# DHDev0/Stochastic-muzero

Hardware: AMD Instinct MI355X
Metric: MCTS simulations/sec (whole node), CartPole MLP 4096 envs × 50 sims (higher is better)
Workload: dtype f32 (tree values, heads) + f64 (pUCT scores, root priors) + i32 (counts)

## Files before the change

stochastic-muzero_amd/csrc/smz_kernels.hip:

```cpp
#ifndef SMZ_SEARCH_THREADS
#define SMZ_SEARCH_THREADS 512
#endif
#ifndef SMZ_EB_WAVES
#define SMZ_EB_WAVES 4
#endif
#ifndef SMZ_PAIR_K4
#define SMZ_PAIR_K4 1
#endif
#ifndef SMZ_KS4
#define SMZ_KS4 1
#endif
#ifndef SMZ_PART
#define SMZ_PART 0
#endif
#ifndef SMZ_PRIO_TREE
#define SMZ_PRIO_TREE 0
#define SMZ_PRIO_HEADS 3
#endif
#include <hip/hip_runtime.h>
#include <math.h>
#include <stdint.h>
#include <stdio.h>
#include <stdlib.h>
#include <string.h>
// ... 582 lines not shown
        r[0] = (double)(float)nx; r[1] = (double)(float)nxd; r[2] = (double)(float)nth; r[3] = (double)(float)nthd;
        r[4] = 1.0;
        r[5] = (double)flag;
        r[6] = policy[(size_t)e * A]; r[7] = policy[(size_t)e * A + 1];
        r[8] = act == 0 ? 1.0 : 0.0; r[9] = act == 1 ? 1.0 : 0.0;
        r[10] = (double)root_value[e];
        r[11] = child_visits[(size_t)e * A]; r[12] = child_visits[(size_t)e * A + 1];
    }
    if (E.reward_out) E.reward_out[e] = 1.0f;
    if (E.flag_out) E.flag_out[e] = (uint8_t)flag;
    int next_count = count;
    if (flag != 0 && E.on_end == 2) {
        const int ep = E.episode[e] + 1;
        E.episode[e] = ep;
        nx = -0.05 + 0.1 * smz_unit(E.reset_seed, (uint64_t)(E.first_env + e), (uint64_t)ep, 0);
        nxd = -0.05 + 0.1 * smz_unit(E.reset_seed, (uint64_t)(E.first_env + e), (uint64_t)ep, 1);
        nth = -0.05 + 0.1 * smz_unit(E.reset_seed, (uint64_t)(E.first_env + e), (uint64_t)ep, 2);
        nthd = -0.05 + 0.1 * smz_unit(E.reset_seed, (uint64_t)(E.first_env + e), (uint64_t)ep, 3);
        next_count = 0;
    } else if (flag != 0 && E.on_end == 1 && E.active) {
        E.active[e] = 0;
    }
    if (E.step_count) E.step_count[e] = next_count;
    st[0] = nx; st[1] = nxd; st[2] = nth; st[3] = nthd;
    if (E.obs_out) {
        float *o = E.obs_out + (size_t)e * 4;
        o[0] = (float)nx; o[1] = (float)nxd; o[2] = (float)nth; o[3] = (float)nthd;
    }
}

extern __shared__ float4 smz_search_lds4[];

#ifndef SMZ_BPS_HBM
#define SMZ_BPS_HBM 1
#endif
#ifndef SMZ_SELECT_BLOCKS
#define SMZ_SELECT_BLOCKS 1
#endif
#ifndef SMZ_EARLY_ROWS
#define SMZ_EARLY_ROWS 1
#endif
#ifndef SMZ_PAIR_A4
#define SMZ_PAIR_A4 1
#endif
#ifndef SMZ_SELECT_TWO_PASSES
#define SMZ_SELECT_TWO_PASSES 1
#endif
#ifndef SMZ_LEAF_FIRST
#define SMZ_LEAF_FIRST 1
#endif
#ifndef SMZ_EARLY_STAGE
#define SMZ_EARLY_STAGE 1
#endif
#ifdef SMZ_BPS_PROBE
#define SMZ_PROBE_DECL unsigned long long pb_t0 = 0, pb_acc[7] = {0, 0, 0, 0, 0, 0, 0};
#define SMZ_PROBE_START pb_t0 = __builtin_amdgcn_s_memtime();
#define SMZ_PROBE_AT(i) { const unsigned long long pb_t1 = __builtin_amdgcn_s_memtime(); pb_acc[i] += pb_t1 - pb_t0; pb_t0 = pb_t1; }
#if SMZ_BPS_PROBE + 0 == 2
#define SMZ_PROBE(i)
#define SMZ_PROBE_B(i) SMZ_PROBE_AT(i)
#else
#define SMZ_PROBE(i) SMZ_PROBE_AT(i)
#define SMZ_PROBE_B(i)
#endif
#define SMZ_PROBE_FLUSH(stats) if ((stats) && lane == 0) { for (int pb_i = 0; pb_i < 7; pb_i++) atomicAdd(&(stats)[8 + pb_i], pb_acc[pb_i]); }
#else
#define SMZ_PROBE_DECL
#define SMZ_PROBE_START
#define SMZ_PROBE(i)
#define SMZ_PROBE_B(i)
#define SMZ_PROBE_FLUSH(stats)
#endif

struct MegaLds {
    int pbc_off, wave_off, per_wave;
    int x_off, pv_off, rng_off, out_off, sel_off, sel_n;
    int sel_on;
    int trees_off, tree_words;
};
__host__ __device__ inline int r4(int x) { return (x + 3) & ~3; }
__host__ __device__ inline MegaLds mega_lds(const smz_mlp_desc &d, const Params &P, int tpw, bool tlds = false, int waves = 8) {
    MegaLds m;
    m.pbc_off = r4(tlds ? smz_mlp::compact_total_floats(d) : d.total_floats - smz_mlp::rep_floats(d));
    m.wave_off = m.pbc_off + r4(2 * 2 * (P.sims + 2));
    m.x_off = r4(2 * smz_mlp::row_scratch_floats(d));
    m.pv_off = m.x_off + tpw * smz_mlp::up4(P.S + P.A);
    m.rng_off = m.pv_off + tpw * P.P * 4;
    m.out_off = m.rng_off + r4(tpw * kRngStride);
    m.sel_off = m.out_off + r4(tpw * (P.A + 2));
    m.sel_n = (P.sims + 2 + 1) & ~1;
    bool sel = tlds;
    if (!tlds && SMZ_BPS_HBM && P.A == 2 && P.K == 2 && tpw == 2 && P.sims <= 126) {
        const int per = m.sel_off + r4(tpw * m.sel_n);
        sel = ((size_t)m.wave_off + (size_t)waves * per) * sizeof(float) <= (size_t)160 * 1024;
    }
    m.sel_on = sel ? 1 : 0;
    m.per_wave = m.sel_off + (sel ? r4(tpw * m.sel_n) : 0);
    m.tree_words = r4(P.rb_words + P.sims * 6 * P.K + (P.K == 2 ? 2 * P.sims : 0));
    m.trees_off = m.wave_off + waves * m.per_wave;
    return m;
}

struct ActOut {
    double temperature;
    int32_t *action;
    double *policy, *child_visits;
    float *root_value;
};
constexpr int kFastTpw = 2, kFastS = 31, kFastH = 64, kFastL = 0;
#if SMZ_PART == 0 || SMZ_PART == 2 || SMZ_PART == 4 || SMZ_PART == 6
template <int MAXA, int KS, int U, bool INSTR, bool AEX, bool MSK = true, bool PHX = false, bool TLDS = false>
__global__ void __launch_bounds__(SMZ_SEARCH_THREADS) k_search_mlp(Params Pin, smz_mlp_desc d, const float *weights, const float *obs,
                                                    int train, ActOut act, EnvStep env) {
    Params P = Pin;
    P.tree0 = 0;
    if (AEX) { P.A = MAXA; P.tpw = kFastTpw; d.A = MAXA; d.S = kFastS; d.H = kFastH; d.L = kFastL; d.OP = smz_mlp::kWave; P.S = kFastS; }
    if (AEX) P.philox = PHX ? 1 : 0;
    if (KS > 0) P.K = KS;
    fix_layout(P, AEX, KS > 0);
    if (AEX) P.hs = (kFastS + 15) & ~15;
    float *lds = reinterpret_cast<float *>(smz_search_lds4);
    static_assert(!TLDS || (AEX && KS > 0), "LDS-resident trees: the specialised instantiations only");
    const smz_mlp_desc dl = TLDS ? smz_mlp::lds_desc_compact(d) : smz_mlp::lds_desc_without_rep(d);
    if (TLDS) smz_mlp::stage_weights_compact(lds, weights, d);
    else smz_mlp::stage_weights_without_rep(lds, weights, d);
    const int lane = threadIdx.x & (kWave - 1), wave = threadIdx.x / kWave, waves = blockDim.x / kWave;
    const int A = P.A, S = P.S, tpw = P.tpw;
    const MegaLds ml = mega_lds(d, P, tpw, TLDS, waves);
    uint32_t *const nodes_global = P.nodes;
    const int gl_eb_words = P.eb_words;
    if (TLDS) {
        uint32_t *nodes_lds = reinterpret_cast<uint32_t *>(lds + ml.trees_off);
        for (int i = threadIdx.x; i < waves * tpw * ml.tree_words; i += blockDim.x) nodes_lds[i] = 0u;
        P.nodes = nodes_lds;
        P.tree0 = blockIdx.x * waves * tpw;
        P.eb_words = 6 * KS;
        P.tree_words = ml.tree_words;
    }
    constexpr bool THR = AEX && KS == 2, YV = THR && TLDS;
    if (THR) {
        P.thr_off = TLDS ? P.rb_words + P.sims * 6 * KS : P.rb_words + 12;
        P.thr_stride = TLDS ? 2 : P.eb_words;
        P.ry_off = (YV && MAXA <= 8 && P.rp_off + 3 * A <= P.rb_words) ? P.rp_off + 2 * A : -1;
    }
    double *pbc_lds = reinterpret_cast<double *>(lds + ml.pbc_off);
    const int n_pbc = P.sims + 2;
    for (int i = threadIdx.x; i < n_pbc; i += blockDim.x) {
        pbc_lds[i] = P.pbc_sqrt[i];
        pbc_lds[n_pbc + i] = i > 0 ? 1.0 / (double)i : 0.0;
    }
    const int slot = A + 2;
    const int K4in = smz_mlp::up4(S + A);
    float *scratch = lds + ml.wave_off + wave * ml.per_wave;
    float *xall = scratch + ml.x_off;
    uint4 *pvals = reinterpret_cast<uint4 *>(scratch + ml.pv_off);
    uint32_t *rng_tile = reinterpret_cast<uint32_t *>(scratch + ml.rng_off);
    float *outs = scratch + ml.out_off;
    __syncthreads();

    const int tree0 = (blockIdx.x * waves + wave) * tpw;
    const int tree = tree0 + lane;
    const bool valid = lane < tpw && tree < P.B && (!MSK || tree_active(P, tree));
    if (MSK && __ballot(valid) == 0ull) {
        if (env.state && lane < tpw && tree < P.B) cartpole_env_step(env, tree, P.B, act.action, act.policy, act.child_visits, act.root_value);
        return;
    }

    for (int t = 0; t < tpw; t++) {
        const int row = tree0 + t;
        if (row >= P.B) break;
        if (MSK && !__shfl((int)valid, t)) continue;
        smz_mlp::initial_row<U, TLDS>(lds, dl, weights, d, scratch, obs + (size_t)row * d.obs, P.hidden + (size_t)row * P.N * P.hs,
                                      nullptr, outs + t * slot);
    }
    constexpr bool PHC = !AEX || PHX;
    int packed = wave_stage_rng<PHC>(P, tree, valid, rng_tile);
    RngT<PHC> rng;
    rng.bind(P, tree, valid);
    TreeHdr h = {0, 0, 0.f, 0.f, 0, 0.f, 0, 0};
    if (valid) {
        rng.load(P.mt + (size_t)tree * kMtN, packed, rng_tile + lane * kRngStride, kRngStage);
        root_init_tree<MAXA>(P, tree, rng, outs + lane * slot, nullptr, train != 0);
        h = P.hdr[tree];
        packed = rng.pack();
    }
    unsigned n_dec = 0, n_chance = 0, n_children = 0, n_desc = 0;
    const int vmask = MSK ? __builtin_amdgcn_readlane((int)valid, 0) | (__builtin_amdgcn_readlane((int)valid, 1) << 1) : 3;
#define SMZ_SLOT_VALID(src) (MSK ? ((vmask >> (src)) & 1) != 0 : tree0 + (src) < P.B)
    const bool prof = INSTR && (P.dbg & 16) && P.stats;
    const int dbg = INSTR ? P.dbg : 0;
    unsigned long long t_stage = 0, t_expand = 0, t_select = 0, t_mlp = 0, t0 = 0, t1 = 0;
#define SMZ_STAMP(acc) if (INSTR && prof) { t1 = __builtin_amdgcn_s_memtime(); acc += t1 - t0; t0 = t1; }
    constexpr int SU = 2;
    const bool split = P.tpw <= SU;
    if (P.sims > 0 && !(dbg & 8)) packed = wave_stage_rng_from<4, PHC>(P, tree, valid, rng_tile, packed, rng.block());
    SMZ_PROBE_DECL
    for (int s = 0; s < P.sims; s++) {
        if (INSTR && prof) t0 = __builtin_amdgcn_s_memtime();
        SMZ_PROBE_START
        Leaf L = {0, 0, 0, 0};
        __builtin_amdgcn_s_setprio(SMZ_PRIO_TREE);
        constexpr bool LBKP = AEX && !INSTR;
        float leaf_rw = 0.f;
        if (valid) {
            rng.load(P.mt + (size_t)tree * kMtN, packed, rng_tile + lane * kRngStride, kRngStage);
            if (s > 0 && !(dbg & 4)) expand_backup_tree<MAXA, KS, LBKP, THR, YV>(P, tree, rng, h, outs + lane * slot, outs[lane * slot + A + 1],
                                                      outs[lane * slot + A], pvals + lane * P.P, &leaf_rw);
        }
        SMZ_PROBE_B(0)
        if constexpr (LBKP) {
            if (s > 0) {
                const int src = lane & (kFastTpw - 1);
                const int len = pick_lane01(h.path_len, src);
                const float lrw = pick_lane01(leaf_rw, src);
                if (lane < 8 * kFastTpw && SMZ_SLOT_VALID(src)) {
                    const bool own = lane < kFastTpw;
                    float mn = own ? h.mn : __builtin_inff(), mx = own ? h.mx : -__builtin_inff(), v_root = 0.f;
                    backup_levels_lanes<kFastTpw, YV>(P, tree0 + src, lane / kFastTpw, len, outs[src * slot + A], lrw,
                                                  pvals + src * P.P, mn, mx, v_root);
                    if (own) {
                        const float nvs = h.root_value_sum + v_root;
                        const int nvc = h.root_visit + 1;
                        h.root_value_sum = nvs;
                        h.root_visit = nvc;
                        const float qv = nvs / (float)nvc;
                        if (qv > mx) mx = qv;
                        if (qv < mn) mn = qv;
                        h.mn = mn;
                        h.mx = mx;
                    }
                }
            }
        }
        SMZ_STAMP(t_expand)
        SMZ_PROBE(0)
        SMZ_PROBE_B(1)
        constexpr bool PAIR = AEX && (MAXA == 2 || (SMZ_PAIR_A4 && MAXA == 4)) && (KS == 2 || (SMZ_PAIR_K4 && KS == 4 && MAXA == 4)) && !INSTR;
        constexpr bool BPS = SMZ_SELECT_BLOCKS && AEX && KS == 2 && (TLDS || SMZ_BPS_HBM) && !INSTR && MAXA == 2;
// ... 162 lines not shown
            if (tree0 + 1 < P.B) {
                const float *xin[2] = {xall, xall + K4in};
                const bool dyn[2] = {b0 != 0, b1 != 0};
                float *dh[2], *dp[2] = {outs, outs + slot};
                float reward[2], value[2];
#pragma unroll
                for (int r = 0; r < 2; r++)
                    dh[r] = P.hidden + ((size_t)(tree0 + r) * P.N + __builtin_amdgcn_readlane(L.leaf_id, r)) * P.hs;
                const bool live[2] = {MSK ? (vmask & 1) != 0 : true, MSK ? (vmask & 2) != 0 : true};
                if (b0 == b1) smz_mlp::recurrent_rows<U, 2, true, TLDS>(lds, dl, scratch, xin, dyn, live, dh, dp, reward, value);
                else smz_mlp::recurrent_rows<U, 2, false, TLDS>(lds, dl, scratch, xin, dyn, live, dh, dp, reward, value);
                SMZ_PROBE_B(4)
                if (lane == 0) {
                    outs[A] = value[0]; outs[A + 1] = reward[0];
                    outs[slot + A] = value[1]; outs[slot + A + 1] = reward[1];
                }
                paired = true;
            }
        }
        for (int t = 0; t < tpw && !paired; t += smz_mlp::kRows) {
            if (tree0 + t >= P.B) break;
            constexpr int R = smz_mlp::kRows;
            const float *xin[R];
            bool dyn[R], live[R];
            float *dh[R], *dp[R];
            float reward[R], value[R];
#pragma unroll
            for (int r = 0; r < R; r++) {
                live[r] = (t + r < tpw) && (tree0 + t + r < P.B);
                const int tt = live[r] ? t + r : t;
                live[r] = live[r] && (!MSK || __shfl((int)valid, tt) != 0);
                const int row = tree0 + tt;
                const int leaf = __builtin_amdgcn_readlane(L.leaf_id, tt);
                dyn[r] = __builtin_amdgcn_readlane(L.branch, tt) != 0;
                xin[r] = xall + tt * K4in;
                dh[r] = P.hidden + ((size_t)row * P.N + leaf) * P.hs;
                dp[r] = outs + tt * slot;
            }
            if (!(dbg & 1)) smz_mlp::recurrent_rows<U, R, false, TLDS>(lds, dl, scratch, xin, dyn, live, dh, dp, reward, value);
#pragma unroll
            for (int r = 0; r < R; r++)
                if (live[r] && lane == 0) { outs[(t + r) * slot + A] = value[r]; outs[(t + r) * slot + A + 1] = reward[r]; }
        }
        smz_mlp::lds_sync();
        SMZ_STAMP(t_mlp)
        SMZ_PROBE(5)
        SMZ_PROBE_B(5)
        if (!(dbg & 8)) packed = split ? stage_finish<SU, PHC>(P, tree, valid, rng_tile, packed, pre, rng.block())
                                       : wave_stage_rng_from<4, PHC>(P, tree, valid, rng_tile, packed, rng.block());
        SMZ_STAMP(t_stage)
        SMZ_PROBE(6)
        SMZ_PROBE_B(6)
    }
    SMZ_PROBE_FLUSH(Pin.stats)
#undef SMZ_STAMP
#undef SMZ_SLOT_VALID
    if (INSTR && prof && lane == 0) {
        atomicAdd(&P.stats[4], t_stage); atomicAdd(&P.stats[5], t_expand);
        atomicAdd(&P.stats[6], t_select); atomicAdd(&P.stats[7], t_mlp);
    }
    if (valid) {
        if (P.sims > 0) {
            rng.load(P.mt + (size_t)tree * kMtN, packed, rng_tile + lane * kRngStride, kRngStage);
            expand_backup_tree<MAXA, KS, false, THR, YV>(P, tree, rng, h, outs + lane * slot, outs[lane * slot + A + 1], outs[lane * slot + A],
                                                     pvals + lane * P.P);
            for (int i = 0; i < h.path_len; i++) P.path[(size_t)i * P.B + tree] = pvals[lane * P.P + i];
            packed = rng.pack();
        }
        P.hdr[tree] = h;
        if (act.action) {
            act_tree<MAXA>(P, tree, rng, act.temperature, act.action, act.policy, act.child_visits, act.root_value);
            packed = rng.pack();
        }
        P.rng_pos[tree] = packed;
        rng.save(P, tree);
    }
    if constexpr (TLDS) {
        smz_mlp::lds_sync();
        const int n_blk = 1 + P.sims;
        for (int t = 0; t < tpw; t++) {
            if (tree0 + t >= P.B) break;
            if (MSK && !__shfl((int)valid, t)) continue;
            const uint32_t *src = P.nodes + (size_t)(wave * tpw + t) * P.tree_words;
            uint32_t *dst = nodes_global + (size_t)(tree0 + t) * (P.rb_words + (size_t)P.sims * gl_eb_words);
            for (int i = lane; i < P.rb_words; i += kWave) dst[i] = src[i];
            for (int i = lane; i < (n_blk - 1) * gl_eb_words; i += kWave) {
                const int b = i / gl_eb_words, w = i - b * gl_eb_words;
                dst[P.rb_words + i] = w < P.eb_words ? src[P.rb_words + b * P.eb_words + w] : 0u;
            }
        }
    }
    if (env.state && lane < tpw && tree < P.B)
        cartpole_env_step(env, tree, P.B, act.action, act.policy, act.child_visits, act.root_value);
    if (INSTR) wave_add_stats(P.stats, n_dec, n_chance, n_desc, n_children);
}
#endif

#if SMZ_PART != 2 && SMZ_PART != 4 && SMZ_PART != 5 && SMZ_PART != 6
__global__ void __launch_bounds__(kWave) k_root_stats(Params P, int32_t *visits, double *priors, float *root_value,
                                                      float *child_reward) {
    const int tree = blockIdx.x * kWave + threadIdx.x;
    if (tree >= P.B) return;
    const uint32_t *rb = tree_base(P, tree);
    const double *rp = (const double *)(rb + P.rp_off);
    for (int a = 0; a < P.A; a++) {
        if (visits) visits[(size_t)tree * P.A + a] = (int32_t)rb[2 * a];
        if (priors) priors[(size_t)tree * P.A + a] = rp[a];
        if (child_reward) child_reward[(size_t)tree * P.A + a] = __uint_as_float(rb[2 * P.A + a]);
    }
    if (root_value) {
        const TreeHdr h = P.hdr[tree];
        root_value[tree] = h.root_visit ? h.root_value_sum / (float)h.root_visit : 0.0f;
    }
}
#endif

#if SMZ_PART != 2 && SMZ_PART != 4 && SMZ_PART != 5 && SMZ_PART != 6
template <int MAXA>
__global__ void __launch_bounds__(kWave) k_act(Params P, double temperature, int32_t *action, double *policy,
                                               double *child_visits, float *root_value) {
    const int tree = blockIdx.x * kWave + threadIdx.x;
    if (tree >= P.B || !tree_active(P, tree)) return;
    Rng rng;
    rng.bind(P, tree, true);
    rng.load(P.mt + (size_t)tree * kMtN, P.rng_pos[tree], nullptr, 0);
    act_tree<MAXA>(P, tree, rng, temperature, action, policy, child_visits, root_value);
    P.rng_pos[tree] = rng.pack();
    rng.save(P, tree);
}
#endif

__device__ inline float grp_max(float v, int lpr) {
    for (int off = lpr >> 1; off > 0; off >>= 1) v = fmaxf(v, __shfl_xor(v, off));
    return v;
}
__device__ inline float grp_min(float v, int lpr) {
    for (int off = lpr >> 1; off > 0; off >>= 1) v = fminf(v, __shfl_xor(v, off));
    return v;
}
__device__ inline float grp_sum(float v, int lpr) {
    for (int off = lpr >> 1; off > 0; off >>= 1) v += __shfl_xor(v, off);
    return v;
}

__device__ inline float support_decode_group(const float *row, int S, int li, int lpr) {
    float m = -__builtin_inff();
// ... 390 lines not shown
    HIP_TRY(hipGetDeviceCount(&ndev));
    if (cfg->device < 0 || cfg->device >= ndev) return fail(SMZ_ERR_INVALID, "device ordinal out of range%s");
    DeviceGuard guard(cfg->device);

    smz_handle *h = new (std::nothrow) smz_handle();
    if (!h) return fail(SMZ_ERR_NOMEM, "host allocation failed%s");
    h->cfg = *cfg;
    const int B = cfg->num_trees, A = cfg->num_actions, S = cfg->hidden_size, sims = cfg->num_simulations;
    h->K = cfg->max_action_sample < A ? cfg->max_action_sample : A;
    h->N = 1 + A + sims * h->K;
    h->Ppath = sims + 2;
    h->maxa = A <= 2 ? 2 : A <= 4 ? 4 : A <= 8 ? 8 : A <= 16 ? 16 : 32;
    h->root_ready = h->selected = false;
    h->pow_valid = false;
    h->d_player_neg = nullptr;
    h->large_actions = large_actions;
    h->pow_T = 0.0;
    h->stats_on = false;

    Params &P = h->P;
    memset(&P, 0, sizeof(P));
    P.B = B; P.A = A; P.K = h->K; P.S = S; P.N = h->N; P.P = h->Ppath; P.sims = sims;
    P.dbg = getenv("SMZ_DEBUG_SKIP") ? atoi(getenv("SMZ_DEBUG_SKIP")) : 0;
    {
        int tpw = kWave;
        while (tpw > 1 && (B + tpw - 1) / tpw < 1024) tpw >>= 1;
        if (const char *e = getenv("SMZ_TREES_PER_WAVE")) {
            const int v = atoi(e);
            if (v == 1 || v == 2 || v == 4 || v == 8 || v == 16 || v == 32 || v == 64) tpw = v;
        }
        P.tpw = tpw;
        P.lds_stage = 1;
        if (const char *e = getenv("SMZ_LDS_STAGE")) P.lds_stage = atoi(e) ? 1 : 0;
    }
    P.disc32 = (float)cfg->discount;
    P.keep32 = (float)(1.0 - cfg->root_exploration_fraction);
    P.frac = cfg->root_exploration_fraction;
    P.alpha = cfg->root_dirichlet_alpha;
    const size_t BN = (size_t)B * h->N;
    P.rp_off = (5 * A + 1) & ~1;
    P.rb_words = ((P.rp_off + 2 * A) + 15) & ~15;
    P.eb_words = ((6 * h->K) + 15) & ~15;
    P.tree_words = (int64_t)P.rb_words + (int64_t)sims * P.eb_words;
    int rc = SMZ_OK;
    auto A_ = [&](int r) { if (rc == SMZ_OK) rc = r; };
    A_(dev_alloc(h, &P.nodes, (size_t)B * (size_t)P.tree_words));
    P.hs = (S + 15) & ~15;
    A_(dev_alloc(h, &P.hidden, BN * (size_t)P.hs));
    A_(dev_alloc(h, &P.hdr, (size_t)B));
    A_(dev_alloc(h, &P.path, (size_t)B * h->Ppath));
    A_(dev_alloc(h, &P.mt, (size_t)B * kMtN));
    A_(dev_alloc(h, &P.rng_pos, (size_t)B));
    A_(dev_alloc(h, &h->d_seeds, (size_t)B));
    A_(dev_alloc(h, &h->d_pbc, (size_t)sims + 2));
    A_(dev_alloc(h, &h->d_pow, (size_t)sims + 1));
    A_(dev_alloc(h, &h->d_stats, (size_t)16));
    A_(dev_alloc(h, &h->d_mt_backup, (size_t)B * kMtN));
    A_(dev_alloc(h, &h->d_pos_backup, (size_t)B));
    A_(dev_alloc(h, &h->d_block_backup, (size_t)B));
    {
        uint32_t *key = nullptr;
        A_(dev_alloc(h, &P.rng_block, (size_t)B));
        A_(dev_alloc(h, &key, (size_t)2 * B));
        P.rng_key = key;
    }
    P.philox = cfg->rng_mode == SMZ_RNG_PHILOX ? 1 : 0;
    h->has_backup = false;
    h->last_kernel[0] = 0;
    if (rc != SMZ_OK) { smz_destroy(h); return rc; }
    P.pbc_sqrt = h->d_pbc;
    P.pow_table = nullptr;
    P.stats = nullptr;
    hipError_t e = hipMemset(P.nodes, 0, (size_t)B * (size_t)P.tree_words * sizeof(uint32_t));
    if (e == hipSuccess) e = hipMemset(P.hdr, 0, (size_t)B * sizeof(TreeHdr));
    if (e == hipSuccess) e = hipMemset(h->d_stats, 0, 16 * sizeof(unsigned long long));
    if (e == hipSuccess) e = hipMemset(P.rng_pos, 0, (size_t)B * sizeof(int32_t));
    if (e == hipSuccess) e = hipMemset(P.mt, 0, (size_t)B * kMtN * sizeof(uint32_t));
    if (e == hipSuccess) e = hipMemset(P.rng_block, 0, (size_t)B * sizeof(uint32_t));
    if (e == hipSuccess) e = hipMemset(const_cast<uint32_t *>(P.rng_key), 0, (size_t)2 * B * sizeof(uint32_t));
    if (e != hipSuccess) { smz_destroy(h); return fail(SMZ_ERR_HIP, "hipMemset failed: %s", hipGetErrorString(e)); }
    std::vector<double> tab((size_t)sims + 2);
    for (int n = 0; n < sims + 2; n++)
        tab[n] = log(((double)n + (double)cfg->pb_c_base + 1.0) / (double)cfg->pb_c_base) + cfg->pb_c_init;
    rc = smz_set_pb_c_table(h, tab.data(), sims + 2);
    if (rc != SMZ_OK) { smz_destroy(h); return rc; }
    std::vector<uint64_t> seeds((size_t)B);
    for (int i = 0; i < B; i++) seeds[i] = (uint64_t)i;
    rc = smz_seed(h, seeds.data(), nullptr);
    if (rc == SMZ_OK) { e = hipDeviceSynchronize(); if (e != hipSuccess) rc = fail(SMZ_ERR_HIP, "sync failed: %s", hipGetErrorString(e)); }
    if (rc != SMZ_OK) { smz_destroy(h); return rc; }
    *out = h;
    return SMZ_OK;
}
}

extern "C" {
int smz_destroy(smz_handle *h) {
    if (!h) return SMZ_OK;
    DeviceGuard guard(h->cfg.device);
    (void)hipDeviceSynchronize();
    for (void *p : h->allocs) (void)hipFree(p);
    delete h;
    return SMZ_OK;
}

int smz_set_pb_c_table(smz_handle *h, const double *host_table, int n) {
    if (!h || !host_table) return fail(SMZ_ERR_INVALID, "smz_set_pb_c_table: null argument%s");
    const int need = h->cfg.num_simulations + 2;
    if (n < need) return fail(SMZ_ERR_INVALID, "smz_set_pb_c_table: table shorter than num_simulations + 2%s");
    DeviceGuard guard(h->cfg.device);
    std::vector<double> t((size_t)need);
    for (int i = 0; i < need; i++) t[i] = sqrt((double)i) * host_table[i];
    HIP_TRY(hipDeviceSynchronize());
    HIP_TRY(hipMemcpy(h->d_pbc, t.data(), (size_t)need * sizeof(double), hipMemcpyHostToDevice));
    return SMZ_OK;
}

int smz_seed(smz_handle *h, const uint64_t *host_seeds, smz_stream stream) {
    if (!h || !host_seeds) return fail(SMZ_ERR_INVALID, "smz_seed: null argument%s");
    DeviceGuard guard(h->cfg.device);
    hipStream_t s = (hipStream_t)stream;
    HIP_TRY(hipStreamSynchronize(s));
    HIP_TRY(hipMemcpy(h->d_seeds, host_seeds, (size_t)h->cfg.num_trees * sizeof(uint64_t), hipMemcpyHostToDevice));
    hipLaunchKernelGGL(k_seed, tree_grid(h->P.B), dim3(kWave), 0, s, h->P, h->d_seeds);
    return launch_check();
}

int smz_set_rng_state(smz_handle *h, int tree, const uint32_t *host_key, int pos) {
    if (!h || !host_key || tree < 0 || tree >= h->cfg.num_trees || pos < 0 || pos > kMtN)
        return fail(SMZ_ERR_INVALID, "smz_set_rng_state: bad argument%s");
    if (h->P.philox) return fail(SMZ_ERR_STATE, "smz_set_rng_state: numpy (MT19937) states belong to SMZ_RNG_MT19937_NUMPY handles%s");
    DeviceGuard guard(h->cfg.device);
    HIP_TRY(hipDeviceSynchronize());
    HIP_TRY(hipMemcpy(h->P.mt + (size_t)tree * kMtN, host_key, kMtN * sizeof(uint32_t), hipMemcpyHostToDevice));
    const int32_t packed = (pos == kMtN) ? 0 : (((kMtN - pos) << 16) | pos);
    HIP_TRY(hipMemcpy(h->P.rng_pos + tree, &packed, sizeof(int32_t), hipMemcpyHostToDevice));
    return SMZ_OK;
}

int smz_get_rng_state(smz_handle *h, int tree, uint32_t *host_key, int *pos) {
    if (!h || !host_key || !pos || tree < 0 || tree >= h->cfg.num_trees)
        return fail(SMZ_ERR_INVALID, "smz_get_rng_state: bad argument%s");
    if (h->P.philox) return fail(SMZ_ERR_STATE, "smz_get_rng_state: numpy (MT19937) states belong to SMZ_RNG_MT19937_NUMPY handles%s");
    DeviceGuard guard(h->cfg.device);
    HIP_TRY(hipDeviceSynchronize());
    int32_t packed = 0;
    HIP_TRY(hipMemcpy(host_key, h->P.mt + (size_t)tree * kMtN, kMtN * sizeof(uint32_t), hipMemcpyDeviceToHost));
    HIP_TRY(hipMemcpy(&packed, h->P.rng_pos + tree, sizeof(int32_t), hipMemcpyDeviceToHost));
    const int idx = packed & 0xffff, ready = packed >> 16;
    auto twist_at = [&](int i) {
        const int i1 = (i + 1 == kMtN) ? 0 : i + 1;
        int im = i + kMtM;
        if (im >= kMtN) im -= kMtN;
        const uint32_t t = (host_key[i] & 0x80000000u) | (host_key[i1] & 0x7fffffffu);
        host_key[i] = host_key[im] ^ (t >> 1) ^ ((t & 1u) ? 0x9908b0dfu : 0u);
    };
    if (idx + ready <= kMtN) {
        if (idx == 0 && ready == 0) { *pos = kMtN; return SMZ_OK; }
        for (int i = idx + ready; i < kMtN; i++) twist_at(i);
        *pos = idx;
        return SMZ_OK;
    }
    const int w = idx + ready - kMtN;
    if (w + kMtM > kMtN) return fail(SMZ_ERR_STATE, "smz_get_rng_state: twist-ahead window too long%s");
    std::vector<uint32_t> t((size_t)w);
    for (int k = 0; k < w; k++) {
        uint32_t y = host_key[k] ^ host_key[k + kMtM];
// ... 692 lines not shown
        std::vector<uint4> recs((size_t)hdr.path_len);
        HIP_TRY(hipMemcpy2D(recs.data(), sizeof(uint4), P.path + tree, (size_t)P.B * sizeof(uint4), sizeof(uint4), (size_t)hdr.path_len, hipMemcpyDeviceToHost));
        path_out[0] = 0;
        const int sb = h->large_actions ? 10 : 8;
        for (int i = 0; i < hdr.path_len && i + 1 < cap_path; i++) {
            const int blk = (int)recs[i].x >> sb, slot = (int)recs[i].x & ((1 << sb) - 1);
            path_out[i + 1] = blk == 0 ? 1 + slot : 1 + A + (blk - 1) * K + slot;
        }
    }
    if (root_priors_out) memcpy(root_priors_out, blob.data() + P.rp_off, (size_t)A * 8);
    return n;
}

int smz_philox_words(uint64_t seed, uint32_t block, int idx, int n, uint32_t *host_out) {
    if (!host_out || n < 0 || idx < 0 || idx >= kMtN) return fail(SMZ_ERR_INVALID, "smz_philox_words: bad argument%s");
    for (int i = 0; i < n; i++) {
        host_out[i] = philox_word(block, idx, (uint32_t)(seed & 0xffffffffull), (uint32_t)(seed >> 32));
        if (++idx == kMtN) { idx = 0; ++block; }
    }
    return SMZ_OK;
}

int smz_get_philox_position(smz_handle *h, int tree, uint32_t *block_out, int *idx_out) {
    if (!h || tree < 0 || tree >= h->cfg.num_trees || !block_out || !idx_out)
        return fail(SMZ_ERR_INVALID, "smz_get_philox_position: bad argument%s");
    if (!h->P.philox) return fail(SMZ_ERR_STATE, "smz_get_philox_position: the handle draws from MT19937%s");
    DeviceGuard guard(h->cfg.device);
    HIP_TRY(hipDeviceSynchronize());
    int32_t packed = 0;
    HIP_TRY(hipMemcpy(&packed, h->P.rng_pos + tree, sizeof(int32_t), hipMemcpyDeviceToHost));
    HIP_TRY(hipMemcpy(block_out, h->P.rng_block + tree, sizeof(uint32_t), hipMemcpyDeviceToHost));
    *idx_out = packed & 0xffff;
    return SMZ_OK;
}

int smz_enable_stats(smz_handle *h, int on) {
    if (!h) return fail(SMZ_ERR_INVALID, "smz_enable_stats: null handle%s");
    if (h->large_actions && on)
        return fail(SMZ_ERR_TOO_LARGE, "smz_enable_stats: the large-action kernels keep no level statistics%s");
    h->stats_on = on != 0;
    h->P.stats = h->stats_on ? h->d_stats : nullptr;
    return SMZ_OK;
}

int smz_read_stats(smz_handle *h, uint64_t levels_out[4], int reset) {
    if (!h || !levels_out) return fail(SMZ_ERR_INVALID, "smz_read_stats: null argument%s");
    DeviceGuard guard(h->cfg.device);
    HIP_TRY(hipDeviceSynchronize());
    unsigned long long v[16];
    HIP_TRY(hipMemcpy(v, h->d_stats, sizeof(v), hipMemcpyDeviceToHost));
    for (int i = 0; i < 4; i++) levels_out[i] = (uint64_t)v[i];
    if (getenv("SMZ_DEBUG_SKIP") && (atoi(getenv("SMZ_DEBUG_SKIP")) & 16))
        fprintf(stderr, "[smz phase cycles, summed over waves] stage %llu expand %llu select %llu mlp %llu  (k_search_vision: tree, conv, wait, towers+tails)\n", v[4], v[5], v[6], v[7]);
#ifdef SMZ_BPS_PROBE
    if (v[8])
        fprintf(stderr, "[smz k_search_mlp probe, cycles summed over waves] expand+backup %llu | select: prepare %llu evaluate %llu chase %llu records+leaf %llu "
                        "| networks %llu | staging %llu\n", v[8], v[9], v[10], v[11], v[12], v[13], v[14]);
#endif
    if (getenv("SMZ_DEBUG_SKIP") && (atoi(getenv("SMZ_DEBUG_SKIP")) & 16) && v[8])
        fprintf(stderr, "[smz k_search_vision phases] tree %llu load %llu conv_transition %llu conv_prediction %llu wait %llu layer1 %llu hidden_out %llu tails_stage %llu\n",
                v[8], v[9], v[10], v[11], v[12], v[13], v[14], v[15]);
    if (reset) HIP_TRY(hipMemset(h->d_stats, 0, sizeof(v)));
    return SMZ_OK;
}

#endif

}
```

stochastic-muzero_amd/csrc/smz_mlp_device.hpp:

```cpp
#pragma once
#include <hip/hip_runtime.h>
#include <math.h>
#include <stdint.h>

#include "../../include/smz.h"

namespace smz_mlp {

constexpr int kWave = 64;
enum { M_DYN_IN, M_ADY_IN, M_DYN_MID, M_ADY_MID, M_DYN_OUT, M_ADY_OUT, M_PRE_IN, M_APR_IN, M_PRE_MID, M_APR_MID,
       M_PRE_OUT, M_APR_OUT, M_REP_IN, M_REP_MID, M_REP_OUT, M_COUNT };

__host__ __device__ inline int up4(int x) { return (x + 3) & ~3; }

typedef float v2f __attribute__((ext_vector_type(2)));
__device__ inline v2f pk_fma(float wx, float wy, float ax, float ay, v2f c) {
    v2f w = {wx, wy}, a = {ax, ay};
    return __builtin_elementwise_fma(w, a, c);
}
template <int U, int R, bool SAME = false>
__device__ inline void dense(const float *const (&W)[R], const float *const (&bias)[R], const float *const (&act)[R], int K4,
                             const int (&OP)[R], int lane, float (&acc)[R][U]) {
    const float4 *a4[R], *w4[R];
    v2f acc2[R][U];
// ... 615 lines not shown
            reward[0] = dyn[0] ? r0 : 0.f;
            reward[1] = dyn[1] ? r1 : 0.f;
        } else if (S <= 32 && A <= 32) {
            softmax_decode_pair(acc[0][0], acc[1][0], A, S, lane, live[0] ? dst_policy[0] : nullptr, live[1] ? dst_policy[1] : nullptr,
                                value[0], value[1]);
        } else {
#pragma unroll
            for (int r = 0; r < R; r++) value[r] = softmax_decode_lanes<U>(acc[r], A, S, lane, live[r] ? dst_policy[r] : nullptr);
        }
    } else {
#pragma unroll
    for (int r = 0; r < R; r++) {
        value[r] = softmax_decode_lanes<U>(acc[r], A, S, lane, live[r] ? dst_policy[r] : nullptr);
    }
    }
    lds_sync();
}

template <int U, bool CP = false>
__device__ inline void initial_row(const float *lds, const smz_mlp_desc &d, const float *rep, const smz_mlp_desc &drep,
                                   float *scratch, const float *obs_row, float *dst_hidden0, float *dst_hidden1,
                                   float *dst_policy) {
    const int S = d.S, A = d.A, K4o = up4(d.obs), K4h = up4(d.H), K4s = up4(S);
    const int lane = threadIdx.x & (kWave - 1);
    const int rs = row_scratch_floats(d), kin = rs - K4h - K4s;
    float *xbuf = scratch;
    float *tA[1] = {scratch + kin};
    float *hbuf = tA[0] + K4h;
    for (int k = lane; k < K4o; k += kWave) xbuf[k] = (k < d.obs) ? obs_row[k] : 0.f;
    for (int k = lane; k < K4s; k += kWave) hbuf[k] = 0.f;
    lds_sync();
    const MatOff mi[1] = {pick(drep, true, M_REP_IN, M_REP_IN)}, mm[1] = {pick(drep, true, M_REP_MID, M_REP_MID)};
    const float *xi[1] = {xbuf};
    trunk<U, 1>(rep, drep, mi, mm, xi, K4o, tA, lane);
    float acc[1][U];
    {
        const float *W[1] = {rep + drep.off[M_REP_OUT]}, *Bv[1] = {rep + drep.off[M_COUNT + M_REP_OUT]}, *Ac[1] = {tA[0]};
        dense<U, 1>(W, Bv, Ac, K4h, d.OP, lane, acc);
    }
    scale_lanes<U>(acc[0], 0, S, lane, hbuf, dst_hidden0, dst_hidden1);
    lds_sync();
    const MatOff pi[1] = {pick<CP>(d, true, M_PRE_IN, M_PRE_IN)}, pm[1] = {pick<CP>(d, true, M_PRE_MID, M_PRE_MID)};
    const float *hi[1] = {hbuf};
    trunk<U, 1>(lds, d, pi, pm, hi, K4s, tA, lane);
    {
        const MatOff po = pick<CP>(d, true, M_PRE_OUT, M_PRE_OUT);
        const float *W[1] = {lds + po.w}, *Bv[1] = {lds + po.b}, *Ac[1] = {tA[0]};
        dense<U, 1>(W, Bv, Ac, K4h, po.op, lane, acc);
    }
    softmax_lanes<U>(acc[0], A, lane, dst_policy);
    lds_sync();
}

__host__ __device__ inline int rep_floats(const smz_mlp_desc &d) { return d.off[M_COUNT] - d.off[M_REP_IN]; }
__host__ __device__ inline smz_mlp_desc lds_desc_without_rep(const smz_mlp_desc &d) {
    smz_mlp_desc l = d;
    const int rs = rep_floats(d);
    for (int m = 0; m < M_COUNT; m++) l.off[M_COUNT + m] = d.off[M_COUNT + m] - rs;
    l.total_floats = d.total_floats - rs;
    return l;
}
__device__ inline void stage_weights_without_rep(float *lds, const float *weights, const smz_mlp_desc &d) {
    constexpr int UB = 8;
    const int n_mat = d.off[M_REP_IN], n_bias = d.total_floats - d.off[M_COUNT], rs = rep_floats(d);
    for (int pass = 0; pass < 2; pass++) {
        const float *src = pass ? weights + d.off[M_COUNT] : weights;
        float *dst = pass ? lds + d.off[M_COUNT] - rs : lds;
        const int cnt = pass ? n_bias : n_mat;
        for (int i0 = threadIdx.x * 4; i0 < cnt; i0 += blockDim.x * 4 * UB) {
            float4 v[UB];
#pragma unroll
            for (int u = 0; u < UB; u++) { const int i = i0 + u * blockDim.x * 4; v[u] = *reinterpret_cast<const float4 *>(src + (i < cnt ? i : i0)); }
#pragma unroll
            for (int u = 0; u < UB; u++) { const int i = i0 + u * blockDim.x * 4; if (i < cnt) *reinterpret_cast<float4 *>(dst + i) = v[u]; }
        }
    }
    __syncthreads();
}

__host__ __device__ inline int compact_matrix_floats(const smz_mlp_desc &d) { return mat_off<true>(d, M_REP_IN); }
__host__ __device__ inline int compact_total_floats(const smz_mlp_desc &d) { return compact_matrix_floats(d) + (d.total_floats - d.off[M_COUNT]); }
__device__ inline smz_mlp_desc lds_desc_compact(const smz_mlp_desc &d) {
    smz_mlp_desc l = d;
    l.off[M_COUNT] = compact_matrix_floats(d);
    l.total_floats = compact_total_floats(d);
    return l;
}
__device__ inline void stage_weights_compact(float *lds, const float *weights, const smz_mlp_desc &d) {
    const int kin = up4(d.S + d.A), kmid = d.L > 0 ? up4(d.H) : 0, kh = up4(d.H), ks = up4(d.S);
    const int K[M_REP_IN] = {kin, kin, kmid, kmid, kh, kh, ks, ks, kmid, kmid, kh, kh};
    int dst = 0;
#pragma unroll
    for (int m = 0; m < M_REP_IN; m++) {
        const int op = mat_op<true>(d, m), groups = K[m] >> 2, per = op;
        const float4 *src = reinterpret_cast<const float4 *>(weights + d.off[m]);
        float4 *out = reinterpret_cast<float4 *>(lds + dst);
        for (int i = threadIdx.x; i < groups * per; i += blockDim.x) {
            const int g = i / per, o = i - g * per;
            out[i] = src[g * d.OP + o];
        }
        dst += K[m] * op;
    }
    const int n_bias = d.total_floats - d.off[M_COUNT];
    for (int i = threadIdx.x * 4; i < n_bias; i += blockDim.x * 4)
        *reinterpret_cast<float4 *>(lds + dst + i) = *reinterpret_cast<const float4 *>(weights + d.off[M_COUNT] + i);
    __syncthreads();
// ... 21 lines not shown
```

Measured before the change: 512.4 million.

## Pair root network rows, precompute reciprocals on host, vectorise tree zeroing and write-back

The root representation and prediction networks for the two trees in a wave now run as a single two-row pass (initial_rows, with a pair softmax). Before, they ran as two sequential single-row passes, so weight reads are now shared between the rows. The 1/i reciprocal table is computed on the host and copied in with the pUCT table, so the kernel no longer does double-precision divides. LDS tree zeroing and the global tree write-back use uint4 accesses, and the write-back pads each 12-word edge block to 16 words with zeros. A fixed-part timing probe mode is also added, enabled only when SMZ_BPS_PROBE is 3.

```diff
diff --git a/stochastic-muzero_amd/csrc/smz_kernels.hip b/stochastic-muzero_amd/csrc/smz_kernels.hip
--- a/stochastic-muzero_amd/csrc/smz_kernels.hip
+++ b/stochastic-muzero_amd/csrc/smz_kernels.hip
@@ -658,11 +658,36 @@
 #ifndef SMZ_EARLY_STAGE
 #define SMZ_EARLY_STAGE 1
 #endif
+#ifndef SMZ_ROOT_PAIR
+#define SMZ_ROOT_PAIR 1
+#endif
+#ifndef SMZ_HOST_RECIPROCALS
+#define SMZ_HOST_RECIPROCALS 1
+#endif
+#ifndef SMZ_WRITEBACK_VEC
+#define SMZ_WRITEBACK_VEC 1
+#endif
+#if defined(SMZ_BPS_PROBE) && SMZ_BPS_PROBE + 0 == 3
+#define SMZ_FPROBE_DECL unsigned long long pb_t0 = __builtin_amdgcn_s_memtime(), pb_acc[7] = {0, 0, 0, 0, 0, 0, 0};
+#define SMZ_FPROBE(i) SMZ_PROBE_AT(i)
+#else
+#define SMZ_FPROBE_DECL
+#define SMZ_FPROBE(i)
+#endif
 #ifdef SMZ_BPS_PROBE
+#if SMZ_BPS_PROBE + 0 == 3
+#define SMZ_PROBE_DECL
+#else
 #define SMZ_PROBE_DECL unsigned long long pb_t0 = 0, pb_acc[7] = {0, 0, 0, 0, 0, 0, 0};
+#endif
 #define SMZ_PROBE_START pb_t0 = __builtin_amdgcn_s_memtime();
 #define SMZ_PROBE_AT(i) { const unsigned long long pb_t1 = __builtin_amdgcn_s_memtime(); pb_acc[i] += pb_t1 - pb_t0; pb_t0 = pb_t1; }
-#if SMZ_BPS_PROBE + 0 == 2
+#if SMZ_BPS_PROBE + 0 == 3
+#define SMZ_PROBE(i)
+#define SMZ_PROBE_B(i)
+#undef SMZ_PROBE_START
+#define SMZ_PROBE_START
+#elif SMZ_BPS_PROBE + 0 == 2
 #define SMZ_PROBE(i)
 #define SMZ_PROBE_B(i) SMZ_PROBE_AT(i)
 #else
@@ -718,6 +743,7 @@
 template <int MAXA, int KS, int U, bool INSTR, bool AEX, bool MSK = true, bool PHX = false, bool TLDS = false>
 __global__ void __launch_bounds__(SMZ_SEARCH_THREADS) k_search_mlp(Params Pin, smz_mlp_desc d, const float *weights, const float *obs,
                                                     int train, ActOut act, EnvStep env) {
+    SMZ_FPROBE_DECL
     Params P = Pin;
     P.tree0 = 0;
     if (AEX) { P.A = MAXA; P.tpw = kFastTpw; d.A = MAXA; d.S = kFastS; d.H = kFastH; d.L = kFastL; d.OP = smz_mlp::kWave; P.S = kFastS; }
@@ -737,6 +763,10 @@
     const int gl_eb_words = P.eb_words;
     if (TLDS) {
         uint32_t *nodes_lds = reinterpret_cast<uint32_t *>(lds + ml.trees_off);
+        if (SMZ_WRITEBACK_VEC) {
+            uint4 *z4 = reinterpret_cast<uint4 *>(nodes_lds);
+            for (int i = threadIdx.x; i < waves * tpw * (ml.tree_words >> 2); i += blockDim.x) z4[i] = make_uint4(0u, 0u, 0u, 0u);
+        } else
         for (int i = threadIdx.x; i < waves * tpw * ml.tree_words; i += blockDim.x) nodes_lds[i] = 0u;
         P.nodes = nodes_lds;
         P.tree0 = blockIdx.x * waves * tpw;
@@ -751,6 +781,9 @@
     }
     double *pbc_lds = reinterpret_cast<double *>(lds + ml.pbc_off);
     const int n_pbc = P.sims + 2;
+    if (SMZ_HOST_RECIPROCALS) {
+        for (int i = threadIdx.x; i < 2 * n_pbc; i += blockDim.x) pbc_lds[i] = P.pbc_sqrt[i];
+    } else
     for (int i = threadIdx.x; i < n_pbc; i += blockDim.x) {
         pbc_lds[i] = P.pbc_sqrt[i];
         pbc_lds[n_pbc + i] = i > 0 ? 1.0 / (double)i : 0.0;
@@ -772,6 +805,14 @@
         return;
     }
 
+    SMZ_FPROBE(0)
+    const bool root_pair = SMZ_ROOT_PAIR && tpw == 2 && tree0 + 1 < P.B && (!MSK || __ballot(valid) == 3ull);
+    if (root_pair) {
+        const float *orow[2] = {obs + (size_t)tree0 * d.obs, obs + (size_t)(tree0 + 1) * d.obs};
+        float *hrow[2] = {P.hidden + (size_t)tree0 * P.N * P.hs, P.hidden + (size_t)(tree0 + 1) * P.N * P.hs};
+        float *prow[2] = {outs, outs + slot};
+        smz_mlp::initial_rows<U, TLDS>(lds, dl, weights, d, scratch, orow, hrow, prow);
+    } else
     for (int t = 0; t < tpw; t++) {
         const int row = tree0 + t;
         if (row >= P.B) break;
@@ -779,6 +820,7 @@
         smz_mlp::initial_row<U, TLDS>(lds, dl, weights, d, scratch, obs + (size_t)row * d.obs, P.hidden + (size_t)row * P.N * P.hs,
                                       nullptr, outs + t * slot);
     }
+    SMZ_FPROBE(1)
     constexpr bool PHC = !AEX || PHX;
     int packed = wave_stage_rng<PHC>(P, tree, valid, rng_tile);
     RngT<PHC> rng;
@@ -790,6 +832,7 @@
         h = P.hdr[tree];
         packed = rng.pack();
     }
+    SMZ_FPROBE(2)
     unsigned n_dec = 0, n_chance = 0, n_children = 0, n_desc = 0;
     const int vmask = MSK ? __builtin_amdgcn_readlane((int)valid, 0) | (__builtin_amdgcn_readlane((int)valid, 1) << 1) : 3;
 #define SMZ_SLOT_VALID(src) (MSK ? ((vmask >> (src)) & 1) != 0 : tree0 + (src) < P.B)
@@ -1058,7 +1101,10 @@
         SMZ_PROBE(6)
         SMZ_PROBE_B(6)
     }
+    SMZ_FPROBE(3)
+#if !(defined(SMZ_BPS_PROBE) && SMZ_BPS_PROBE + 0 == 3)
     SMZ_PROBE_FLUSH(Pin.stats)
+#endif
 #undef SMZ_STAMP
 #undef SMZ_SLOT_VALID
     if (INSTR && prof && lane == 0) {
@@ -1081,6 +1127,7 @@
         P.rng_pos[tree] = packed;
         rng.save(P, tree);
     }
+    SMZ_FPROBE(4)
     if constexpr (TLDS) {
         smz_mlp::lds_sync();
         const int n_blk = 1 + P.sims;
@@ -1089,6 +1136,17 @@
             if (MSK && !__shfl((int)valid, t)) continue;
             const uint32_t *src = P.nodes + (size_t)(wave * tpw + t) * P.tree_words;
             uint32_t *dst = nodes_global + (size_t)(tree0 + t) * (P.rb_words + (size_t)P.sims * gl_eb_words);
+            if (SMZ_WRITEBACK_VEC && KS == 2 && gl_eb_words == 16) {
+                const uint4 *src4 = reinterpret_cast<const uint4 *>(src);
+                uint4 *dst4 = reinterpret_cast<uint4 *>(dst);
+                const int rb4 = P.rb_words >> 2;
+                for (int i = lane; i < rb4; i += kWave) dst4[i] = src4[i];
+                for (int i = lane; i < (n_blk - 1) * 4; i += kWave) {
+                    const int b = i >> 2, q = i & 3;
+                    dst4[rb4 + i] = q < 3 ? src4[rb4 + b * 3 + q] : make_uint4(0u, 0u, 0u, 0u);
+                }
+                continue;
+            }
             for (int i = lane; i < P.rb_words; i += kWave) dst[i] = src[i];
             for (int i = lane; i < (n_blk - 1) * gl_eb_words; i += kWave) {
                 const int b = i / gl_eb_words, w = i - b * gl_eb_words;
@@ -1096,8 +1154,13 @@
             }
         }
     }
+    SMZ_FPROBE(5)
     if (env.state && lane < tpw && tree < P.B)
         cartpole_env_step(env, tree, P.B, act.action, act.policy, act.child_visits, act.root_value);
+    SMZ_FPROBE(6)
+#if defined(SMZ_BPS_PROBE) && SMZ_BPS_PROBE + 0 == 3
+    SMZ_PROBE_FLUSH(Pin.stats)
+#endif
     if (INSTR) wave_add_stats(P.stats, n_dec, n_chance, n_desc, n_children);
 }
 #endif
@@ -1594,7 +1657,7 @@
     A_(dev_alloc(h, &P.mt, (size_t)B * kMtN));
     A_(dev_alloc(h, &P.rng_pos, (size_t)B));
     A_(dev_alloc(h, &h->d_seeds, (size_t)B));
-    A_(dev_alloc(h, &h->d_pbc, (size_t)sims + 2));
+    A_(dev_alloc(h, &h->d_pbc, 2 * ((size_t)sims + 2)));
     A_(dev_alloc(h, &h->d_pow, (size_t)sims + 1));
     A_(dev_alloc(h, &h->d_stats, (size_t)16));
     A_(dev_alloc(h, &h->d_mt_backup, (size_t)B * kMtN));
@@ -1651,10 +1714,13 @@
     const int need = h->cfg.num_simulations + 2;
     if (n < need) return fail(SMZ_ERR_INVALID, "smz_set_pb_c_table: table shorter than num_simulations + 2%s");
     DeviceGuard guard(h->cfg.device);
-    std::vector<double> t((size_t)need);
-    for (int i = 0; i < need; i++) t[i] = sqrt((double)i) * host_table[i];
+    std::vector<double> t((size_t)2 * need);
+    for (int i = 0; i < need; i++) {
+        t[i] = sqrt((double)i) * host_table[i];
+        t[need + i] = i > 0 ? 1.0 / (double)i : 0.0;
+    }
     HIP_TRY(hipDeviceSynchronize());
-    HIP_TRY(hipMemcpy(h->d_pbc, t.data(), (size_t)need * sizeof(double), hipMemcpyHostToDevice));
+    HIP_TRY(hipMemcpy(h->d_pbc, t.data(), (size_t)2 * need * sizeof(double), hipMemcpyHostToDevice));
     return SMZ_OK;
 }
 
@@ -2453,7 +2519,11 @@
     for (int i = 0; i < 4; i++) levels_out[i] = (uint64_t)v[i];
     if (getenv("SMZ_DEBUG_SKIP") && (atoi(getenv("SMZ_DEBUG_SKIP")) & 16))
         fprintf(stderr, "[smz phase cycles, summed over waves] stage %llu expand %llu select %llu mlp %llu  (k_search_vision: tree, conv, wait, towers+tails)\n", v[4], v[5], v[6], v[7]);
-#ifdef SMZ_BPS_PROBE
+#if defined(SMZ_BPS_PROBE) && SMZ_BPS_PROBE + 0 == 3
+    if (v[8])
+        fprintf(stderr, "[smz k_search_mlp fixed-part probe, cycles summed over waves] staging+tables+zeroing %llu | root networks %llu | root expansion+noise %llu "
+                        "| rounds %llu | last expansion+act %llu | write-back %llu | env step %llu\n", v[8], v[9], v[10], v[11], v[12], v[13], v[14]);
+#elif defined(SMZ_BPS_PROBE)
     if (v[8])
         fprintf(stderr, "[smz k_search_mlp probe, cycles summed over waves] expand+backup %llu | select: prepare %llu evaluate %llu chase %llu records+leaf %llu "
                         "| networks %llu | staging %llu\n", v[8], v[9], v[10], v[11], v[12], v[13], v[14]);
diff --git a/stochastic-muzero_amd/csrc/smz_mlp_device.hpp b/stochastic-muzero_amd/csrc/smz_mlp_device.hpp
--- a/stochastic-muzero_amd/csrc/smz_mlp_device.hpp
+++ b/stochastic-muzero_amd/csrc/smz_mlp_device.hpp
@@ -691,6 +691,75 @@
     lds_sync();
 }
 
+__device__ inline void softmax_pair(float a0, float a1, int A, int lane, float *dst0, float *dst1) {
+    float P = a0, Q = a1;
+    swap32(P, Q);
+    const bool hi = lane >= 32;
+    const int j = lane & 31;
+    const bool in = j < A;
+    float m = in ? P : -__builtin_inff(), m2 = m;
+    half_max2(m, m2);
+    m = half_bcast(m, hi);
+    const float e = in ? smz_exp(P - m) : 0.f;
+    float den = e, den2 = e;
+    half_sum2(den, den2);
+    den = half_bcast(den, hi);
+    float *dst = hi ? dst1 : dst0;
+    if (in) dst[j] = __fdividef(e, den);
+}
+
+template <int U, bool CP = false>
+__device__ inline void initial_rows(const float *lds, const smz_mlp_desc &d, const float *rep, const smz_mlp_desc &drep,
+                                    float *scratch, const float *const (&obs_row)[2], float *const (&dst_hidden)[2],
+                                    float *const (&dst_policy)[2]) {
+    constexpr int R = 2;
+    const int S = d.S, A = d.A, K4o = up4(d.obs), K4h = up4(d.H), K4s = up4(S);
+    const int lane = threadIdx.x & (kWave - 1);
+    const int rs = row_scratch_floats(d), kin = rs - K4h - K4s;
+    float *xbuf[R], *tA[R], *hbuf[R];
+#pragma unroll
+    for (int r = 0; r < R; r++) {
+        xbuf[r] = scratch + r * rs;
+        tA[r] = xbuf[r] + kin;
+        hbuf[r] = tA[r] + K4h;
+        for (int k = lane; k < K4o; k += kWave) xbuf[r][k] = (k < d.obs) ? obs_row[r][k] : 0.f;
+        for (int k = lane; k < K4s; k += kWave) hbuf[r][k] = 0.f;
+    }
+    lds_sync();
+    const MatOff mi1 = pick(drep, true, M_REP_IN, M_REP_IN), mm1 = pick(drep, true, M_REP_MID, M_REP_MID);
+    const MatOff mi[R] = {mi1, mi1}, mm[R] = {mm1, mm1};
+    const float *xi[R] = {xbuf[0], xbuf[1]};
+    trunk<U, R, true>(rep, drep, mi, mm, xi, K4o, tA, lane);
+    float acc[R][U];
+    {
+        const float *W[R] = {rep + drep.off[M_REP_OUT], rep + drep.off[M_REP_OUT]};
+        const float *Bv[R] = {rep + drep.off[M_COUNT + M_REP_OUT], rep + drep.off[M_COUNT + M_REP_OUT]}, *Ac[R] = {tA[0], tA[1]};
+        dense<U, R, true>(W, Bv, Ac, K4h, d.OP, lane, acc);
+    }
+    const bool pair_tails = SMZ_PAIR_TAILS && U == 1 && S <= 32 && A <= 32;
+    if (pair_tails) scale_pair(acc[0][0], acc[1][0], S, lane, hbuf[0], hbuf[1], dst_hidden[0], dst_hidden[1]);
+    else {
+#pragma unroll
+        for (int r = 0; r < R; r++) scale_lanes<U>(acc[r], 0, S, lane, hbuf[r], dst_hidden[r]);
+    }
+    lds_sync();
+    const MatOff pi1 = pick<CP>(d, true, M_PRE_IN, M_PRE_IN), pm1 = pick<CP>(d, true, M_PRE_MID, M_PRE_MID);
+    const MatOff pi[R] = {pi1, pi1}, pm[R] = {pm1, pm1};
+    const float *hi[R] = {hbuf[0], hbuf[1]};
+    trunk<U, R, true>(lds, d, pi, pm, hi, K4s, tA, lane);
+    {
+        const MatOff po = pick<CP>(d, true, M_PRE_OUT, M_PRE_OUT);
+        const float *W[R] = {lds + po.w, lds + po.w}, *Bv[R] = {lds + po.b, lds + po.b}, *Ac[R] = {tA[0], tA[1]};
+        dense<U, R, true>(W, Bv, Ac, K4h, po.op, lane, acc);
+    }
+    if (pair_tails) softmax_pair(acc[0][0], acc[1][0], A, lane, dst_policy[0], dst_policy[1]);
+    else {
+#pragma unroll
+        for (int r = 0; r < R; r++) softmax_lanes<U>(acc[r], A, lane, dst_policy[r]);
+    }
+    lds_sync();
+}
+
 __host__ __device__ inline int rep_floats(const smz_mlp_desc &d) { return d.off[M_COUNT] - d.off[M_REP_IN]; }
 __host__ __device__ inline smz_mlp_desc lds_desc_without_rep(const smz_mlp_desc &d) {
     smz_mlp_desc l = d;
```

Result: no change. 512.5 million (median of 2 runs) (+0.0%).
